# welcomyou/sherpa-vietnamese-asr

Measured on AMD Instinct MI355X. Metric: audio-sec/sec (xRT) Zipformer-68M offline decode, higher is better.
Workload: dtype bf16; 1 GPU; zipformer-68m greedy_search, batched planner chunks, 1 h per GPU; model=zipformer-68m, weights=greedy-calibrated, chunks_per_gpu=121, batch_pipeline=True, encoder_frames_per_gpu=98813

## Files before the change

include/zasr.h:

```cpp
#ifndef ZASR_H_
#define ZASR_H_

#include <stdint.h>

#ifdef __cplusplus
extern "C" {
#endif

typedef struct zasr_recognizer zasr_recognizer;
typedef struct zasr_result zasr_result;

enum {
  ZASR_OK = 0,
  ZASR_ERR_INVALID = 1,
  ZASR_ERR_NOT_FOUND = 2,
  ZASR_ERR_RUNTIME = 3,
};

enum {
  ZASR_PRECISION_FP32 = 0,
  ZASR_PRECISION_BF16 = 1,
  ZASR_PRECISION_BF16_ENC = 2,
  ZASR_PRECISION_BF16X3 = 3,
  ZASR_PRECISION_BF16X6 = 4,
// ... 115 lines not shown

typedef struct zasr_audio zasr_audio;
enum { ZASR_AUDIO_F32 = 0, ZASR_AUDIO_I16 = 1 };
int zasr_audio_create(int32_t device_id, zasr_audio** out);
void zasr_audio_destroy(zasr_audio* h);
int64_t zasr_audio_out_len(int32_t rate, int64_t n_frames);
int zasr_audio_resample_taps(int32_t rate, int32_t* P, int32_t* Q, int32_t* taps,
                             int32_t* out_tile, int32_t* in_tile, int32_t* lo, float* w,
                             int64_t cap);
int zasr_audio_to_16k(zasr_audio* h, const void* src, int32_t format, int32_t channels,
                      int32_t rate, int64_t n_frames, int32_t src_on_device, float* d_out,
                      int64_t cap, int64_t* n_out, void* stream);
int zasr_audio_peak(zasr_audio* h, const float* d_wav, int64_t n, float* peak, void* stream);
int zasr_audio_scale(zasr_audio* h, float* d_wav, int64_t n, float divisor, float multiplier,
                     void* stream);
int zasr_audio_segment_sumsq(zasr_audio* h, const float* d_wav, int64_t n,
                             const int64_t* seg_begin, const int64_t* seg_end, int32_t n_seg,
                             double* out, void* stream);
int zasr_audio_apply_gain(zasr_audio* h, float* d_wav, int64_t n, const int64_t* piece_begin,
                          const int64_t* piece_end, const float* piece_gain,
                          const int64_t* piece_ramp, int32_t n_pieces, const float* ramp_values,
                          int64_t n_ramp_values, float* peak, void* stream);

int32_t zasr_vocab_size(const zasr_recognizer* h);
int32_t zasr_joiner_dim(const zasr_recognizer* h);
int zasr_model_routes(zasr_recognizer* h, char* buf, int64_t cap);
int zasr_fbank_set_mel_banks(zasr_recognizer* h, const float* banks, int32_t n_bins);
int zasr_selftest_launch(int32_t block_threads);
int zasr_selftest_gemm_h3r(int32_t M, int32_t K, int32_t N, int32_t epi, const float* A,
                           const float* W, const float* bias, float* C);
int zasr_selftest_ffn_h3(int32_t R, int32_t D, int32_t F, const float* Y, const float* W1,
                         const float* b1, const float* W2, const float* b2,
                         const float* byp_orig, const float* byp_scale, float* X);
int zasr_selftest_gemm(int32_t mode, int32_t M, int32_t K, int32_t N, int32_t epi, int32_t a_bf16,
                       int32_t c_bf16, const float* A, const float* W, const float* bias,
                       const float* aux, const float* byp_orig, const float* byp_scale, float* C);
int zasr_selftest_ffn_bf16(int32_t R, int32_t D, int32_t F, const float* W1, const float* b1,
                           const float* W2, const float* b2, const float* byp_orig,
                           const float* byp_scale, float* X, int32_t form);
int zasr_selftest_ffn_bf16_oop(int32_t R, int32_t D, int32_t F, const float* W1, const float* b1,
                               const float* W2, const float* b2, const float* byp_orig,
                               const float* byp_scale, float* X, float* Xout, int32_t form);
int zasr_selftest_ffn_h3_oop(int32_t R, int32_t D, int32_t F, const float* W1, const float* b1,
                             const float* W2, const float* b2, const float* byp_orig,
                             const float* byp_scale, float* X, float* Xout);
int zasr_selftest_seam(int32_t nseq, const int32_t* L, int32_t d, int32_t ds, int32_t dn,
                       int32_t ds_next, int32_t c0, int32_t ldo, const float* xd,
                       const float* orig, const float* s, const float* wn8, const float* wo2,
                       float* next, float* xnext, float* out, float* next_ref, float* xnext_ref,
                       float* out_ref);
int zasr_selftest_dwconv1d(int32_t nseq, const int32_t* L, int32_t d, int32_t K, int32_t glu,
                           int32_t bf16, const float* x, const float* w, const float* b,
                           float* out);
int zasr_selftest_conv1(int32_t nseq, const int32_t* T, int32_t form, const float* fb,
                        const float* w, const float* b, float* out);
int zasr_selftest_convnext(int32_t nseq, const int32_t* L, int32_t form, const float* x,
                           const float* dw_w, const float* dw_b, const float* w1, const float* b1,
                           const float* w2, const float* b2, float* y, float* out);
int zasr_selftest_bias_norm(int32_t rows, int32_t d, const float* bias, float log_scale,
                            float* orig, const float* bscale, int32_t copy_mode, float* x,
                            float* copy_out);
int zasr_selftest_attn_block_map(const int32_t* lens, int32_t nseq, int32_t units_per_seq,
                                 int32_t order, uint32_t* out, int64_t cap, int32_t* grid);

typedef struct zasr_diar zasr_diar;
int zasr_diar_create(int32_t device_id, zasr_diar** out);
void zasr_diar_destroy(zasr_diar* h);
int zasr_diar_similarity(zasr_diar* h, const float* d_X, int32_t N, int32_t D, float* d_M,
                         void* stream);
int zasr_diar_prune(zasr_diar* h, float* d_M, int32_t N, double pval, int32_t min_pnum,
                    double* d_deg, void* stream);
int zasr_diar_eigs(zasr_diar* h, const float* d_M, const double* d_deg, int32_t N, int32_t k,
                   double* lambdas, double* vecs, int32_t* passes, void* stream);
int zasr_diar_spectral_embed(zasr_diar* h, const float* X, int32_t x_on_device, int32_t N,
                             int32_t D, double pval, int32_t min_pnum, int32_t k,
                             double* lambdas, double* vecs, void* stream);
int zasr_diar_last_stats(zasr_diar* h, int32_t* passes, int64_t* applications);

int zasr_profile_enable(zasr_recognizer* h, int32_t on);
int zasr_profile_reset(zasr_recognizer* h);
int zasr_profile_report(zasr_recognizer* h, char* buf, int64_t cap);

const char* zasr_last_error(void);
const char* zasr_version(void);

#ifdef __cplusplus
}
#endif
#endif
```

sherpa-vietnamese-asr_amd/csrc/encoder_kernels.hip:

```cpp
#include "common.h"
#include "kernels.h"

namespace zasr {

typedef float f32x16 __attribute__((ext_vector_type(16)));

__device__ __forceinline__ int find_seq(const int* off, int nseq, int r) {
  int lo = 0, hi = nseq - 1;
  while (lo < hi) {
    int mid = (lo + hi + 1) >> 1;
    if (off[mid] <= r) lo = mid;
    else hi = mid - 1;
  }
  return lo;
}

__global__ void row2seq_kernel(const int* __restrict__ off, int nseq, int total,
                               int* __restrict__ map) {
  int r = blockIdx.x * blockDim.x + threadIdx.x;
  if (r < total) map[r] = find_seq(off, nseq, r);
}

void launch_row2seq(const int* off, int nseq, int total, int* map, hipStream_t st) {
  if (total <= 0) return;
// ... 532 lines not shown
    }
  }
  if (tid < kDw1T) {
    const int r = r0 + tid;
    int lo = -half, hi = half;
    if (r < total_rows) {
      lo = max(seq_lo - r, -half);
      hi = min(seq_hi - 1 - r, half);
    }
    sLo[tid] = lo;
    sHi[tid] = hi;
    if (lo != -half || hi != half) atomicOr(&sMasked, 1);
  }
  __syncthreads();
  if (c0 + c >= d) return;
  const int tr0 = (tid >> 6) * 16;
  float acc[16];
#pragma unroll
  for (int i = 0; i < 16; ++i) acc[i] = bc;
  if (!sMasked) {
#pragma unroll
    for (int rr = 0; rr < 16 + K - 1; ++rr) {
      const float v = tile[(tr0 + rr) * 64 + c];
#pragma unroll
      for (int i = 0; i < 16; ++i) {
        const int k = rr - i;
        if (k >= 0 && k < K) acc[i] = fmaf(wr[k], v, acc[i]);
      }
    }
  } else {
    int lo[16], hi[16];
#pragma unroll
    for (int i = 0; i < 16; ++i) {
      lo[i] = sLo[tr0 + i];
      hi[i] = sHi[tr0 + i];
    }
#pragma unroll
    for (int rr = 0; rr < 16 + K - 1; ++rr) {
      const float v = tile[(tr0 + rr) * 64 + c];
#pragma unroll
      for (int i = 0; i < 16; ++i) {
        const int k = rr - i;
        if (k >= 0 && k < K && k - half >= lo[i] && k - half <= hi[i]) acc[i] = fmaf(wr[k], v, acc[i]);
      }
    }
  }
#pragma unroll
  for (int i = 0; i < 16; ++i) {
    const int r = r0 + tr0 + i;
    if (r < total_rows) st1(out + (long)r * d + c0 + c, swooshr_fast(acc[i]));
  }
}

template <typename TI, typename TO, bool GLU = true>
static void launch_glu_dwconv1d_t(const TI* x2, const int* off, const int* map, int total_rows,
                                  int d, int K, const float* w, const float* b, TO* out,
                                  hipStream_t st) {
  if (total_rows <= 0) return;
  ZASR_REQUIRE(d % 4 == 0, "conv module channels must be a multiple of 4");
  dim3 grid(cdiv(total_rows, kDw1T), cdiv(d, 64));
  ZASR_REQUIRE(K >= 1 && K <= 31 && (K & 1), "depthwise kernel size must be odd and <= 31");
  if (K <= 7)
    ZASR_LAUNCH((glu_dwconv1d_kernel<7, TI, TO, GLU>), grid, dim3(256), 0, st, x2, off, map, total_rows, d, K, w, b, out);
  else if (K <= 15)
    ZASR_LAUNCH((glu_dwconv1d_kernel<15, TI, TO, GLU>), grid, dim3(256), 0, st, x2, off, map, total_rows, d, K, w, b, out);
  else
    ZASR_LAUNCH((glu_dwconv1d_kernel<31, TI, TO, GLU>), grid, dim3(256), 0, st, x2, off, map, total_rows, d, K, w, b, out);
}

void launch_dwconv1d_post_glu(const float* g, const int* off, const int* map, int total_rows,
                              int d, int K, const float* w, const float* b, float* out,
                              hipStream_t st) {
  launch_glu_dwconv1d_t<float, float, false>(g, off, map, total_rows, d, K, w, b, out, st);
}

void launch_dwconv1d_post_glu_bf16(const void* g, const int* off, const int* map,
                                   int total_rows, int d, int K, const float* w, const float* b,
                                   void* out, hipStream_t st) {
  launch_glu_dwconv1d_t<__bf16, __bf16, false>(reinterpret_cast<const __bf16*>(g), off, map,
                                               total_rows, d, K, w, b,
                                               reinterpret_cast<__bf16*>(out), st);
}

void launch_glu_dwconv1d(const float* x2, const int* off, const int* map, int total_rows, int d,
                         int K, const float* w, const float* b, float* out, hipStream_t st) {
  launch_glu_dwconv1d_t(x2, off, map, total_rows, d, K, w, b, out, st);
}

struct DsW {
  float w[8];
};

template <int DS>
__global__ void downsample_kernel(const float* __restrict__ x, const int* __restrict__ off_in,
                                  const int* __restrict__ off_out, const int* __restrict__ map_out,
                                  int total_out,
                                  int d4, int ds, DsW wts, float* __restrict__ out) {
  const int e = blockIdx.x * blockDim.x + threadIdx.x;
  if (e >= total_out * d4) return;
  const int r = e / d4, c4 = e - r * d4;
  const int b = map_out[r];
  const int tp = r - off_out[b];
  const int base = off_in[b];
  const int L = off_in[b + 1] - base;
  const float4* x4 = reinterpret_cast<const float4*>(x);
  constexpr int NL = DS > 0 ? DS : 8;
  const int f = DS > 0 ? DS : ds;
  float4 xv[NL];
#pragma unroll
  for (int u = 0; u < NL; ++u) {
    int t = tp * f + (u < f ? u : 0);
    if (t > L - 1) t = L - 1;
    xv[u] = x4[(base + t) * d4 + c4];
  }
  float4 acc = make_float4(0.f, 0.f, 0.f, 0.f);
#pragma unroll
  for (int u = 0; u < NL; ++u)
    if (u < f) {
      acc.x = fmaf(wts.w[u], xv[u].x, acc.x);
      acc.y = fmaf(wts.w[u], xv[u].y, acc.y);
      acc.z = fmaf(wts.w[u], xv[u].z, acc.z);
      acc.w = fmaf(wts.w[u], xv[u].w, acc.w);
    }
  reinterpret_cast<float4*>(out)[e] = acc;
}

void launch_downsample(const float* x, const int* off_in, const int* off_out, const int* map_out,
                       int total_out, int d, int ds, const float* w_host8, float* out,
                       hipStream_t st) {
  const long n = (long)total_out * (d / 4);
  if (n <= 0) return;
  ZASR_REQUIRE(d % 4 == 0 && n < (1L << 31), "downsample: width must be a multiple of 4");
  DsW w{};
  for (int i = 0; i < ds && i < 8; ++i) w.w[i] = w_host8[i];
// ... 619 lines not shown
```

sherpa-vietnamese-asr_amd/csrc/kernels.h:

```cpp
#pragma once
#include <cstdint>
#include <vector>

#include <hip/hip_runtime.h>

namespace zasr {

struct FbankTables {
  const double* twiddle;
  const float* window;
  const int* mel_start;
  const int* mel_len;
  const int* mel_woff;
  const float* mel_w;
};
void launch_fbank(const float* wav, const long* wav_off, const int* nsamp, const int* fr_off,
                  int nseq, int total_frames, const FbankTables& tabs, float* out,
                  hipStream_t st, bool campp = false);

void launch_silence_flags(const float* wav, long n, int frame_len, float threshold,
                          unsigned char* flags, hipStream_t st);

void launch_selftest_noop(int block_threads);
void selftest_gemm_h3r(int M, int K, int N, int epi, const float* A, const float* W,
// ... 77 lines not shown
  float* frames;
  int n_files;
};
void launch_vad_maxabs(const float* audio, const long* off, const long* len, int n_files,
                       unsigned* mx, hipStream_t st);
void launch_vad_frames(const VadFramesArgs& a, long n_windows, hipStream_t st);
void launch_vad_mag_im2col(const float* S, int ldS, int bins, int Kp, long n_windows, float* A,
                           hipStream_t st);
void launch_vad_im2col(const float* Y, long N, int T, int C, int stride, int Tout, float* A,
                       hipStream_t st);
struct VadLstmArgs {
  const float* gx;
  const float* whh;
  const float* bhh;
  const float* wd;
  float bd;
  const long* seg_start;
  const int* seg_count;
  const int* seg_warm;
  const float* init;
  float* s_out;
  float* e_out;
  float* probs;
};
void launch_vad_lstm(const VadLstmArgs& a, int n_segments, hipStream_t st);

void launch_conv1(const float* fb, const int* fb_off, const int* c1_off, const int* c1_map,
                  int total_rows, const float* w , const float* b, void* out,
                  bool out_bf16, hipStream_t st, bool fast = false);
void pack_frag32_host(const __bf16* w, int rows, int cols, __bf16* out);
void launch_convnext_bf16(const void* x, const int* L_off, const int* L_map, int total_rows,
                          const float* dw_w, const float* dw_b, const void* w1, const float* b1,
                          const void* w2, const float* b2, void* ytmp, void* out,
                          hipStream_t st);
void launch_convnext_mlp_h3(const float* y, const float* x, long npos, const void* w1p,
                            const float* b1, const void* w2p, const float* b2, float* out,
                            hipStream_t st);
void launch_dwconv2d_tiled(const float* x, const int* L_off, const int* L_map, int total_rows,
                           const float* w, const float* b, float* out, hipStream_t st);

void selftest_seam(int nseq, const int* L, int d, int ds, int dn, int ds_next, int c0, int ldo,
                   const float* xd, const float* orig, const float* s, const float* wn8,
                   const float* wo2, float* next, float* xnext, float* out, float* next_ref,
                   float* xnext_ref, float* out_ref);
void launch_bias_norm(float* x, int rows, int d, const float* bias, float log_scale,
                      const float* orig, const float* bypass_scale, hipStream_t st,
                      float* copy_out = nullptr);
void launch_bypass(float* x, const float* orig, const float* s, long rows, int d, hipStream_t st);
void launch_glu(const float* x2, float* g, long rows, int d, hipStream_t st);
void launch_glu_dwconv1d(const float* x2, const int* off, const int* map, int total_rows, int d,
                         int K, const float* w, const float* b, float* out, hipStream_t st);
void launch_dwconv1d_post_glu(const float* g, const int* off, const int* map, int total_rows,
                              int d, int K, const float* w, const float* b, float* out,
                              hipStream_t st);
void launch_dwconv1d_post_glu_bf16(const void* g, const int* off, const int* map,
                                   int total_rows, int d, int K, const float* w, const float* b,
                                   void* out, hipStream_t st);
void launch_nonlin_prep(const float* h3, float* t1, long rows, int hid, hipStream_t st);
void launch_downsample(const float* x, const int* off_in, const int* off_out, const int* map_out,
                       int total_out, int d, int ds, const float* w_host8, float* out,
                       hipStream_t st);
void launch_upsample_combine(const float* xd, const float* orig, const int* off_in,
                             const int* off_ds, const int* map_in, int total_rows, int d, int ds,
                             const float* s, float* y, hipStream_t st);
void launch_stack_glue(const float* xd, const float* orig, const int* off_in, const int* off_ds,
                       const int* map_in, int rows, int d, int ds, const float* s, float* next,
                       int dn, float* full, int ldf, int c0, hipStream_t st);
struct SeamDesc {
  const float* xd = nullptr;
  const float* orig = nullptr;
  const float* s = nullptr;
  const int* off_in = nullptr;
  const int* off_ds = nullptr;
  const int* off_run = nullptr;
  const int* map_run = nullptr;
  int runs = 0;
  int rows = 0;
  int d = 0, ds = 1;
  float* next = nullptr;
  int dn = 0;
  int ds_next = 1;
  float* xnext = nullptr;
  const float* wn_host8 = nullptr;
  float* out = nullptr;
  const int* off_out = nullptr;
  const float* wo_host2 = nullptr;
  int ldo = 0, c0 = 0;
};
void launch_seam(const SeamDesc& s, hipStream_t st);
void selftest_dwconv1d(int nseq, const int* L, int d, int K, bool glu, bool bf16, const float* x,
                       const float* w, const float* b, float* out);
void selftest_conv1(int nseq, const int* T, int form, const float* fb, const float* w,
                    const float* b, float* out);
void selftest_convnext(int nseq, const int* L, int form, const float* x, const float* dw_w,
                       const float* dw_b, const float* w1, const float* b1, const float* w2,
                       const float* b2, float* y, float* out);
void selftest_bias_norm(int rows, int d, const float* bias, float log_scale, float* orig,
                        const float* bscale, int copy_mode, float* x, float* copy_out);
void launch_row2seq(const int* off, int nseq, int total, int* map, hipStream_t st);
void launch_copy_cols(const float* src, int lds, int c0, float* dst, int ldd, int d0, int ncols,
                      long rows, bool zero_rest, int dst_width, hipStream_t st);

struct AttnArgs {
  const float* qkp;
  int H;
  const float* pos_tab;
  int pmax;
  const int* row_off;
  const long* a_off;
  int nseq;
  int max_len;
  float* attn;
  float* stats;
  int write_heads;
};
void launch_attn_softmax(const AttnArgs& a, hipStream_t st);
struct AttnFlashArgs {
  const void* qkp;
  int H;
  const float* pos_tab;
  int pmax;
  const int* row_off;
  const long* a_off;
  int nseq;
  int max_len;
  void* attn;
  const void* v;
  void* out;
  const float* stats_in;
  float* stats_out;
  int pieces = 1;
  const void* t1t = nullptr;
  const int* o8 = nullptr;
  int ldt = 0;
  int hid = 0;
  const void* y = nullptr;
  int ldy = 0;
  void* z = nullptr;
  const unsigned* map = nullptr;
  int map_len = 0;
};
void launch_attn_flash(const AttnFlashArgs& a, int mode, hipStream_t st);
inline int attn_nonlin_frags(int hid, int pieces) {
  const int nft = (hid + 31) / 32;
// ... 185 lines not shown
```

sherpa-vietnamese-asr_amd/csrc/selftest.cpp:

```cpp
#include <cstring>
#include <memory>
#include <vector>

#include "../../include/zasr.h"
#include "common.h"
#include "dense_gemm.h"
#include "gemm.h"
#include "kernels.h"

namespace zasr {
namespace {
struct DevBuf {
  void* p = nullptr;
  explicit DevBuf(size_t bytes) { ZASR_HIP_CHECK(hipMalloc(&p, bytes > 0 ? bytes : 4)); }
  ~DevBuf() { (void)hipFree(p); }
  template <class T>
  T* as() const { return reinterpret_cast<T*>(p); }
};
void up(DevBuf& d, const void* h, size_t bytes) {
  if (bytes) ZASR_HIP_CHECK(hipMemcpy(d.p, h, bytes, hipMemcpyHostToDevice));
}
}

void selftest_gemm_h3r(int M, int K, int N, int epi, const float* A, const float* W,
// ... 275 lines not shown
  DevBuf d_off, d_map;
  Level(int nseq, const int* len, int cut)
      : off(offsets(nseq, len, cut)), rows(off.back()), d_off(off.size() * 4),
        d_map((size_t)rows * 4) {
    up(d_off, off.data(), off.size() * 4);
    launch_row2seq(d_off.as<int>(), nseq, rows, d_map.as<int>(), nullptr);
  }
  static std::vector<int> offsets(int nseq, const int* len, int cut) {
    ZASR_REQUIRE(nseq >= 1 && len != nullptr, "selftest: at least one sequence");
    std::vector<int> o(nseq + 1, 0);
    for (int b = 0; b < nseq; ++b) {
      ZASR_REQUIRE(len[b] - cut >= 1, "selftest: every sequence needs a frame at every level");
      o[b + 1] = o[b] + len[b] - cut;
    }
    return o;
  }
};

struct OutBuf {
  size_t n, row, eb;
  DevBuf d;
  OutBuf(const float* init, size_t n_, size_t row_, bool h16)
      : n(n_), row(row_), eb(h16 ? 2 : 4), d((n_ + row_) * (h16 ? 2 : 4)) {
    if (h16) up(d, round16(init, n).data(), n * 2);
    else up(d, init, n * 4);
    ZASR_HIP_CHECK(hipMemset(d.as<unsigned char>() + n * eb, 0x5a, row * eb));
  }
  template <class T>
  T* as() const { return d.as<T>(); }
  void down(float* out, const char* what) const {
    std::vector<unsigned char> guard(row * eb);
    ZASR_HIP_CHECK(hipMemcpy(guard.data(), d.as<unsigned char>() + n * eb, guard.size(),
                             hipMemcpyDeviceToHost));
    for (unsigned char g : guard)
      ZASR_REQUIRE(g == 0x5a, std::string("selftest ") + what + ": the kernel wrote past the last row");
    if (n == 0) return;
    if (eb == 2) {
      std::vector<__bf16> h(n);
      ZASR_HIP_CHECK(hipMemcpy(h.data(), d.p, n * 2, hipMemcpyDeviceToHost));
      for (size_t i = 0; i < n; ++i) out[i] = (float)h[i];
    } else {
      ZASR_HIP_CHECK(hipMemcpy(out, d.p, n * 4, hipMemcpyDeviceToHost));
    }
  }
};

void up16(DevBuf& d, const float* h, size_t n, bool h16) {
  if (h16) up(d, round16(h, n).data(), n * 2);
  else up(d, h, n * 4);
}
}

void selftest_dwconv1d(int nseq, const int* L, int d, int K, bool glu, bool bf16, const float* x,
                       const float* w, const float* b, float* out) {
  ZASR_REQUIRE(!(glu && bf16), "selftest dwconv1d: the GLU form is f32 only");
  ZASR_REQUIRE(d >= 4 && d % 4 == 0, "selftest dwconv1d: d a positive multiple of 4");
  ZASR_REQUIRE(K >= 1 && K <= 31 && (K & 1), "selftest dwconv1d: K odd, at most 31");
  Level lv(nseq, L, 0);
  const size_t nx = (size_t)lv.rows * (glu ? 2 * d : d), no = (size_t)lv.rows * d;
  DevBuf dX(nx * (bf16 ? 2 : 4)), dW((size_t)d * K * 4), dB((size_t)d * 4);
  up16(dX, x, nx, bf16);
  up(dW, w, (size_t)d * K * 4);
  up(dB, b, (size_t)d * 4);
  OutBuf o(out, no, d, bf16);
  if (glu)
    launch_glu_dwconv1d(dX.as<float>(), lv.d_off.as<int>(), lv.d_map.as<int>(), lv.rows, d, K,
                        dW.as<float>(), dB.as<float>(), o.as<float>(), nullptr);
  else if (bf16)
    launch_dwconv1d_post_glu_bf16(dX.p, lv.d_off.as<int>(), lv.d_map.as<int>(), lv.rows, d, K,
                                  dW.as<float>(), dB.as<float>(), o.d.p, nullptr);
  else
    launch_dwconv1d_post_glu(dX.as<float>(), lv.d_off.as<int>(), lv.d_map.as<int>(), lv.rows, d, K,
                             dW.as<float>(), dB.as<float>(), o.as<float>(), nullptr);
  ZASR_HIP_CHECK(hipDeviceSynchronize());
  o.down(out, "dwconv1d");
}

void selftest_conv1(int nseq, const int* T, int form, const float* fb, const float* w,
                    const float* b, float* out) {
  ZASR_REQUIRE(form >= 0 && form <= 2, "selftest conv1: form 0 (libm), 1 (fast) or 2 (bf16 out)");
  Level lf(nseq, T, 0), lc(nseq, T, 2);
  DevBuf dF((size_t)lf.rows * 80 * 4), dW(8 * 9 * 4), dB(8 * 4);
  up(dF, fb, (size_t)lf.rows * 80 * 4);
  up(dW, w, 8 * 9 * 4);
  up(dB, b, 8 * 4);
  OutBuf o(out, (size_t)lc.rows * 640, 640, form == 2);
  launch_conv1(dF.as<float>(), lf.d_off.as<int>(), lc.d_off.as<int>(), lc.d_map.as<int>(), lc.rows,
               dW.as<float>(), dB.as<float>(), o.d.p, form == 2, nullptr, form == 1);
  ZASR_HIP_CHECK(hipDeviceSynchronize());
  o.down(out, "conv1");
}

void selftest_convnext(int nseq, const int* L, int form, const float* x, const float* dw_w,
                       const float* dw_b, const float* w1, const float* b1, const float* w2,
                       const float* b2, float* y, float* out) {
  ZASR_REQUIRE(form >= 0 && form <= 2,
               "selftest convnext: form 0 (depthwise f32), 1 (bf16 block) or 2 (f16x3 block)");
  ZASR_REQUIRE(form == 0 || (w1 && b1 && w2 && b2 && out), "selftest convnext: the MLP's operands");
  Level lv(nseq, L, 0);
  constexpr size_t kRow = 19 * 128, kW = 384 * 128;
  const size_t n = (size_t)lv.rows * kRow;
  const bool h16 = form == 1;
  DevBuf dWd(128 * 49 * 4), dBd(128 * 4), d1(2 * kW * 2), d2(2 * kW * 2), db1(384 * 4), db2(128 * 4);
  up(dWd, dw_w, 128 * 49 * 4);
  up(dBd, dw_b, 128 * 4);
  OutBuf oy(y, n, kRow, h16);
  const int *off = lv.d_off.as<int>(), *map = lv.d_map.as<int>();
  if (form == 0) {
    DevBuf dX(n * 4);
    up(dX, x, n * 4);
    launch_dwconv2d_tiled(dX.as<float>(), off, map, lv.rows, dWd.as<float>(), dBd.as<float>(),
                          oy.as<float>(), nullptr);
    ZASR_HIP_CHECK(hipDeviceSynchronize());
    oy.down(y, "convnext");
    return;
  }
  up(db1, b1, 384 * 4);
  up(db2, b2, 128 * 4);
  auto pack = [&](const float* wsrc, int rows, int cols, DevBuf& dst) {
    std::vector<__bf16> img(2 * kW), piece(kW);
    if (h16) {
      pack_frag32_host(round16(wsrc, kW).data(), rows, cols, img.data());
    } else {
      for (int t = 0; t < 2; ++t) {
        for (size_t i = 0; i < kW; ++i) {
          const _Float16 hi = (_Float16)wsrc[i];
// ... 57 lines not shown
```

sherpa-vietnamese-asr_amd/csrc/zasr_api.cpp:

```cpp
#include <cstdio>
#include <cstring>
#include <fstream>
#include <memory>
#include <mutex>
#include <sstream>
#include <string>
#include <vector>

#include "../../include/zasr.h"
#include "audio.h"
#include "campp.h"
#include "common.h"
#include "diar.h"
#include "vad.h"
#include "vibert.h"
#include "engine.h"
#include "host_io.h"
#include "onnx_io.h"

using zasr::Engine;
using zasr::TokenResult;

struct zasr_recognizer {
  std::unique_ptr<Engine> eng;
// ... 672 lines not shown
                           const float* byp_scale, float* X, int32_t form) {
  if (!W1 || !b1 || !W2 || !b2 || !X) return fail(ZASR_ERR_INVALID, "null argument");
  return guarded([&]() {
    zasr::selftest_ffn_bf16(R, D, F, W1, b1, W2, b2, byp_orig, byp_scale, X, form);
    return (int)ZASR_OK;
  });
}

int zasr_selftest_ffn_bf16_oop(int32_t R, int32_t D, int32_t F, const float* W1, const float* b1,
                               const float* W2, const float* b2, const float* byp_orig,
                               const float* byp_scale, float* X, float* Xout, int32_t form) {
  if (!W1 || !b1 || !W2 || !b2 || !X || !Xout) return fail(ZASR_ERR_INVALID, "null argument");
  return guarded([&]() {
    zasr::selftest_ffn_bf16(R, D, F, W1, b1, W2, b2, byp_orig, byp_scale, X, form, Xout);
    return (int)ZASR_OK;
  });
}

int zasr_selftest_ffn_h3_oop(int32_t R, int32_t D, int32_t F, const float* W1, const float* b1,
                             const float* W2, const float* b2, const float* byp_orig,
                             const float* byp_scale, float* X, float* Xout) {
  if (!W1 || !b1 || !W2 || !b2 || !X || !Xout) return fail(ZASR_ERR_INVALID, "null argument");
  return guarded([&]() {
    zasr::selftest_ffn_h3(R, D, F, nullptr, W1, b1, W2, b2, byp_orig, byp_scale, X, Xout);
    return (int)ZASR_OK;
  });
}

int zasr_selftest_seam(int32_t nseq, const int32_t* L, int32_t d, int32_t ds, int32_t dn,
                       int32_t ds_next, int32_t c0, int32_t ldo, const float* xd,
                       const float* orig, const float* s, const float* wn8, const float* wo2,
                       float* next, float* xnext, float* out, float* next_ref, float* xnext_ref,
                       float* out_ref) {
  if (!L || !orig || !wn8 || !wo2 || !next || !xnext || !out || !next_ref || !xnext_ref ||
      !out_ref || (ds > 1 && (!xd || !s)))
    return fail(ZASR_ERR_INVALID, "null argument");
  return guarded([&]() {
    zasr::selftest_seam(nseq, L, d, ds, dn, ds_next, c0, ldo, xd, orig, s, wn8, wo2, next, xnext,
                        out, next_ref, xnext_ref, out_ref);
    return (int)ZASR_OK;
  });
}

int zasr_selftest_dwconv1d(int32_t nseq, const int32_t* L, int32_t d, int32_t K, int32_t glu,
                           int32_t bf16, const float* x, const float* w, const float* b,
                           float* out) {
  if (!L || !x || !w || !b || !out) return fail(ZASR_ERR_INVALID, "null argument");
  return guarded([&]() {
    zasr::selftest_dwconv1d(nseq, L, d, K, glu != 0, bf16 != 0, x, w, b, out);
    return (int)ZASR_OK;
  });
}

int zasr_selftest_conv1(int32_t nseq, const int32_t* T, int32_t form, const float* fb,
                        const float* w, const float* b, float* out) {
  if (!T || !fb || !w || !b || !out) return fail(ZASR_ERR_INVALID, "null argument");
  return guarded([&]() {
    zasr::selftest_conv1(nseq, T, form, fb, w, b, out);
    return (int)ZASR_OK;
  });
}

int zasr_selftest_convnext(int32_t nseq, const int32_t* L, int32_t form, const float* x,
                           const float* dw_w, const float* dw_b, const float* w1, const float* b1,
                           const float* w2, const float* b2, float* y, float* out) {
  if (!L || !x || !dw_w || !dw_b || !y) return fail(ZASR_ERR_INVALID, "null argument");
  return guarded([&]() {
    zasr::selftest_convnext(nseq, L, form, x, dw_w, dw_b, w1, b1, w2, b2, y, out);
    return (int)ZASR_OK;
  });
}

int zasr_selftest_bias_norm(int32_t rows, int32_t d, const float* bias, float log_scale,
                            float* orig, const float* bscale, int32_t copy_mode, float* x,
                            float* copy_out) {
  if (!bias || !x) return fail(ZASR_ERR_INVALID, "null argument");
  return guarded([&]() {
    zasr::selftest_bias_norm(rows, d, bias, log_scale, orig, bscale, copy_mode, x, copy_out);
    return (int)ZASR_OK;
  });
}

int zasr_selftest_attn_block_map(const int32_t* lens, int32_t nseq, int32_t units_per_seq,
                                 int32_t order, uint32_t* out, int64_t cap, int32_t* grid) {
  if (!lens || !grid || (cap > 0 && !out) || cap < 0) return fail(ZASR_ERR_INVALID, "null argument");
  return guarded([&]() {
    std::vector<unsigned> map;
    *grid = zasr::build_attn_block_map(lens, nseq, units_per_seq, order, map);
    if ((int64_t)map.size() > cap) return fail(ZASR_ERR_INVALID, "block map buffer too small");
    std::copy(map.begin(), map.end(), out);
    return (int)ZASR_OK;
  });
}

int zasr_silence_flags(const float* d_wav, int64_t n, int32_t frame_len, float threshold,
                       uint8_t* d_flags, void* stream) {
  if (n < 0 || (n > 0 && (!d_wav || !d_flags))) return fail(ZASR_ERR_INVALID, "null argument");
  return guarded([&]() {
    zasr::launch_silence_flags(d_wav, (long)n, (int)frame_len, threshold, d_flags,
                               reinterpret_cast<hipStream_t>(stream));
    return (int)ZASR_OK;
  });
}

namespace {
int audio_source_error(int32_t format, int32_t channels, int32_t rate) {
// ... 349 lines not shown
```

sherpa-vietnamese-asr_amd/zasr/binding.py:

```python
from __future__ import annotations

import ctypes as C
import dataclasses
import os
from typing import List, Optional, Sequence

import numpy as np

_PKG = os.path.dirname(os.path.dirname(os.path.abspath(__file__)))
DEFAULT_LIB = os.path.join(_PKG, "lib", "libzasr.so")

EXPORTS = (
    "zasr_create", "zasr_destroy", "zasr_convert_model", "zasr_convert_stage_model", "zasr_fbank", "zasr_decode_batch", "zasr_decode_features",
    "zasr_decode_device", "zasr_decode_device_batches", "zasr_encode_features", "zasr_search_encoder_out",
    "zasr_result_count", "zasr_result_num_tokens", "zasr_result_num_frames",
    "zasr_result_tokens", "zasr_result_frames", "zasr_result_log_probs",
    "zasr_result_token_stats", "zasr_result_free", "zasr_vocab_size", "zasr_joiner_dim",
    "zasr_profile_enable", "zasr_profile_reset", "zasr_profile_report", "zasr_last_error",
    "zasr_version", "zasr_campp_create", "zasr_campp_destroy", "zasr_campp_embedding_dim",
    "zasr_campp_fbank", "zasr_campp_embed", "zasr_campp_embed_device", "zasr_campp_windows_device",
    "zasr_vibert_create", "zasr_vibert_destroy", "zasr_vibert_num_labels",
    "zasr_vibert_num_detect", "zasr_vibert_run",
    "zasr_vad_create", "zasr_vad_destroy", "zasr_vad_probs", "zasr_vad_probs_device",
    "zasr_vad_window", "zasr_vad_last_passes", "zasr_silence_flags",
    "zasr_create_stream", "zasr_destroy_stream", "zasr_stream_accept_waveform",
    "zasr_decode_stream", "zasr_decode_streams", "zasr_stream_is_decoded",
    "zasr_stream_num_tokens", "zasr_stream_num_frames", "zasr_stream_tokens",
    "zasr_stream_frames", "zasr_stream_log_probs", "zasr_stream_token_stats",
    "zasr_stream_result_json", "zasr_set_tokens", "zasr_model_routes",
    "zasr_fbank_set_mel_banks", "zasr_selftest_launch", "zasr_decode_host_batches",
    "zasr_selftest_gemm_h3r", "zasr_selftest_ffn_h3", "zasr_selftest_ffn_bf16",
    "zasr_selftest_attn_block_map", "zasr_selftest_seam", "zasr_selftest_ffn_bf16_oop",
    "zasr_selftest_ffn_h3_oop", "zasr_selftest_gemm",
    "zasr_selftest_dwconv1d", "zasr_selftest_conv1", "zasr_selftest_convnext",
    "zasr_selftest_bias_norm",
    "zasr_audio_create", "zasr_audio_destroy", "zasr_audio_out_len", "zasr_audio_resample_taps",
    "zasr_audio_to_16k", "zasr_audio_peak", "zasr_audio_scale", "zasr_audio_segment_sumsq",
    "zasr_audio_apply_gain",
    "zasr_diar_create", "zasr_diar_destroy", "zasr_diar_similarity", "zasr_diar_prune",
    "zasr_diar_eigs", "zasr_diar_spectral_embed", "zasr_diar_last_stats",
)


PRECISIONS = {"fp32": 0, "bf16": 1, "bf16_enc": 2, "bf16x3": 3, "bf16x6": 4, "f16x3": 5}


C_FP = C.POINTER(C.c_float)


class ZasrError(RuntimeError):
    pass


class _Config(C.Structure):
    _fields_ = [
        ("model_dir", C.c_char_p),
        ("decoding_method", C.c_char_p),
        ("max_active_paths", C.c_int32),
        ("blank_penalty", C.c_float),
        ("hotword_tokens", C.POINTER(C.c_int32)),
        ("hotword_lens", C.POINTER(C.c_int32)),
        ("hotword_scores", C.POINTER(C.c_float)),
        ("num_hotwords", C.c_int32),
        ("device_id", C.c_int32),
        ("precision", C.c_int32),
    ]


_lib = None


def load_library(path: Optional[str] = None) -> C.CDLL:
    global _lib
    if _lib is not None and path is None:
        return _lib
    p = path or os.environ.get("ZASR_LIB", DEFAULT_LIB)
    if not os.path.exists(p):
        raise ZasrError(f"libzasr.so not found at {p}; build it with "
                        f"`make -C sherpa-vietnamese-asr_amd/csrc` (or __graft_entry__.build())")
    lib = C.CDLL(p)
    P, I32, I64 = C.c_void_p, C.c_int32, C.c_int64
    fp = C.POINTER(C.c_float)
    lib.zasr_create.argtypes = [C.POINTER(_Config), C.POINTER(P)]
    lib.zasr_create.restype = C.c_int
    lib.zasr_destroy.argtypes = [P]
    lib.zasr_destroy.restype = None
    lib.zasr_convert_model.argtypes = [C.c_char_p, C.c_char_p]
    lib.zasr_convert_model.restype = C.c_int
# ... 90 lines not shown
    lib.zasr_vad_last_passes.restype = I32
    lib.zasr_silence_flags.argtypes = [P, I64, I32, C.c_float, P, P]
    lib.zasr_silence_flags.restype = C.c_int
    lib.zasr_create_stream.argtypes = [P, C.POINTER(P)]
    lib.zasr_create_stream.restype = C.c_int
    lib.zasr_destroy_stream.argtypes = [P]
    lib.zasr_destroy_stream.restype = None
    lib.zasr_stream_accept_waveform.argtypes = [P, I32, fp, I64]
    lib.zasr_stream_accept_waveform.restype = C.c_int
    lib.zasr_decode_stream.argtypes = [P, P]
    lib.zasr_decode_stream.restype = C.c_int
    lib.zasr_decode_streams.argtypes = [P, C.POINTER(P), I32]
    lib.zasr_decode_streams.restype = C.c_int
    for n in ("zasr_stream_is_decoded", "zasr_stream_num_tokens", "zasr_stream_num_frames"):
        getattr(lib, n).argtypes = [P]
        getattr(lib, n).restype = I32
    lib.zasr_stream_tokens.argtypes = [P]
    lib.zasr_stream_tokens.restype = C.POINTER(I32)
    lib.zasr_stream_frames.argtypes = [P]
    lib.zasr_stream_frames.restype = C.POINTER(I32)
    lib.zasr_stream_log_probs.argtypes = [P]
    lib.zasr_stream_log_probs.restype = C.POINTER(C.c_double)
    lib.zasr_stream_token_stats.argtypes = [P]
    lib.zasr_stream_token_stats.restype = fp
    lib.zasr_stream_result_json.argtypes = [P, C.c_char_p, I64, C.POINTER(I64)]
    lib.zasr_stream_result_json.restype = C.c_int
    lib.zasr_set_tokens.argtypes = [P, C.c_char_p]
    lib.zasr_set_tokens.restype = C.c_int
    lib.zasr_model_routes.argtypes = [P, C.c_char_p, I64]
    lib.zasr_model_routes.restype = C.c_int
    lib.zasr_fbank_set_mel_banks.argtypes = [P, fp, I32]
    lib.zasr_fbank_set_mel_banks.restype = C.c_int
    lib.zasr_selftest_launch.argtypes = [I32]
    lib.zasr_selftest_launch.restype = C.c_int
    lib.zasr_selftest_gemm_h3r.argtypes = [I32, I32, I32, I32, fp, fp, fp, fp]
    lib.zasr_selftest_gemm_h3r.restype = C.c_int
    lib.zasr_selftest_gemm.argtypes = [I32] * 7 + [fp] * 7
    lib.zasr_selftest_gemm.restype = C.c_int
    lib.zasr_selftest_ffn_h3.argtypes = [I32, I32, I32, fp, fp, fp, fp, fp, fp, fp, fp]
    lib.zasr_selftest_ffn_h3.restype = C.c_int
    lib.zasr_selftest_ffn_bf16.argtypes = [I32, I32, I32, fp, fp, fp, fp, fp, fp, fp, I32]
    lib.zasr_selftest_ffn_bf16.restype = C.c_int
    lib.zasr_selftest_attn_block_map.argtypes = [C.POINTER(I32), I32, I32, I32,
                                                 C.POINTER(C.c_uint32), I64, C.POINTER(I32)]
    lib.zasr_selftest_attn_block_map.restype = C.c_int
    lib.zasr_selftest_seam.argtypes = [I32, C.POINTER(I32)] + [I32] * 6 + [fp] * 11
    lib.zasr_selftest_seam.restype = C.c_int
    lib.zasr_selftest_ffn_bf16_oop.argtypes = [I32, I32, I32] + [fp] * 8 + [I32]
    lib.zasr_selftest_ffn_bf16_oop.restype = C.c_int
    lib.zasr_selftest_ffn_h3_oop.argtypes = [I32, I32, I32] + [fp] * 8
    lib.zasr_selftest_ffn_h3_oop.restype = C.c_int
    lib.zasr_selftest_dwconv1d.argtypes = [I32, C.POINTER(I32)] + [I32] * 4 + [fp] * 4
    lib.zasr_selftest_dwconv1d.restype = C.c_int
    lib.zasr_selftest_conv1.argtypes = [I32, C.POINTER(I32), I32] + [fp] * 4
    lib.zasr_selftest_conv1.restype = C.c_int
    lib.zasr_selftest_convnext.argtypes = [I32, C.POINTER(I32), I32] + [fp] * 9
    lib.zasr_selftest_convnext.restype = C.c_int
    lib.zasr_selftest_bias_norm.argtypes = [I32, I32, fp, C.c_float, fp, fp, I32, fp, fp]
    lib.zasr_selftest_bias_norm.restype = C.c_int
    lib.zasr_audio_create.argtypes = [I32, C.POINTER(P)]
    lib.zasr_audio_create.restype = C.c_int
    lib.zasr_audio_destroy.argtypes = [P]
    lib.zasr_audio_destroy.restype = None
    lib.zasr_audio_out_len.argtypes = [I32, I64]
    lib.zasr_audio_out_len.restype = I64
    lib.zasr_audio_resample_taps.argtypes = [I32, i32p, i32p, i32p, i32p, i32p, i32p, fp, I64]
    lib.zasr_audio_resample_taps.restype = C.c_int
    lib.zasr_audio_to_16k.argtypes = [P, P, I32, I32, I32, I64, I32, P, I64, i64p, P]
    lib.zasr_audio_to_16k.restype = C.c_int
    lib.zasr_audio_peak.argtypes = [P, P, I64, fp, P]
    lib.zasr_audio_peak.restype = C.c_int
    lib.zasr_audio_scale.argtypes = [P, P, I64, C.c_float, C.c_float, P]
    lib.zasr_audio_scale.restype = C.c_int
    lib.zasr_audio_segment_sumsq.argtypes = [P, P, I64, i64p, i64p, I32, C.POINTER(C.c_double), P]
    lib.zasr_audio_segment_sumsq.restype = C.c_int
    lib.zasr_audio_apply_gain.argtypes = [P, P, I64, i64p, i64p, fp, i64p, I32, fp, I64, fp, P]
    lib.zasr_audio_apply_gain.restype = C.c_int
    dp, DBL = C.POINTER(C.c_double), C.c_double
    lib.zasr_diar_create.argtypes = [I32, C.POINTER(P)]
    lib.zasr_diar_create.restype = C.c_int
    lib.zasr_diar_destroy.argtypes = [P]
    lib.zasr_diar_destroy.restype = None
    lib.zasr_diar_similarity.argtypes = [P, P, I32, I32, P, P]
    lib.zasr_diar_similarity.restype = C.c_int
    lib.zasr_diar_prune.argtypes = [P, P, I32, DBL, I32, P, P]
    lib.zasr_diar_prune.restype = C.c_int
    lib.zasr_diar_eigs.argtypes = [P, P, P, I32, I32, dp, dp, i32p, P]
    lib.zasr_diar_eigs.restype = C.c_int
    lib.zasr_diar_spectral_embed.argtypes = [P, P, I32, I32, I32, DBL, I32, I32, dp, dp, P]
    lib.zasr_diar_spectral_embed.restype = C.c_int
    lib.zasr_diar_last_stats.argtypes = [P, i32p, i64p]
    lib.zasr_diar_last_stats.restype = C.c_int
    if path is None:
        _lib = lib
    return lib


def convert_model(model_dir: str, out_dir: str, lib_path: Optional[str] = None) -> None:
    lib = load_library(lib_path)
    os.makedirs(out_dir, exist_ok=True)
    rc = lib.zasr_convert_model(model_dir.encode(), out_dir.encode())
    if rc != 0:
        msg = lib.zasr_last_error().decode()
        if rc == 2:
            raise FileNotFoundError(msg)
        raise ZasrError(msg)
# ... 93 lines not shown
def selftest_ffn_oop(kind: str, W1, b1, W2, b2, X, byp_orig=None, byp_scale=None, form: int = 0,
                     fill: float = -777.25, lib_path: Optional[str] = None):
    lib = load_library(lib_path)
    W1, b1, W2, b2, X = (_f32(v) for v in (W1, b1, W2, b2, X))
    X = X.copy()
    out = np.full(X.shape, fill, dtype=np.float32)
    bo = None if byp_orig is None else _f32(byp_orig)
    bs = None if byp_scale is None else _f32(byp_scale)
    p = lambda x: None if x is None else x.ctypes.data_as(C_FP)
    args = (X.shape[0], X.shape[1], W1.shape[0], p(W1), p(b1), p(W2), p(b2), p(bo), p(bs), p(X),
            p(out))
    if kind == "bf16":
        rc = lib.zasr_selftest_ffn_bf16_oop(*args, int(form))
    elif kind == "h3":
        rc = lib.zasr_selftest_ffn_h3_oop(*args)
    else:
        raise ValueError(kind)
    if rc != 0:
        raise ZasrError(lib.zasr_last_error().decode())
    return out, X


def selftest_seam(L, d: int, ds: int, dn: int, ds_next: int, c0: int, ldo: int, xd, orig, s,
                  wn8, wo2, fill: float = -777.25, lib_path: Optional[str] = None) -> dict:
    lib = load_library(lib_path)
    L = np.ascontiguousarray(L, dtype=np.int32)
    orig, wn8, wo2 = _f32(orig), _f32(wn8), _f32(wo2)
    xd = None if xd is None else _f32(xd)
    s = None if s is None else _f32(s)
    rows = int(L.sum())
    rn = int(((L + ds_next - 1) // ds_next).sum())
    ro = int(((L + 1) // 2).sum())
    assert orig.shape == (rows, d) and wn8.shape == (8,) and wo2.shape == (2,)
    assert ds == 1 or (xd.shape == (int(((L + ds - 1) // ds).sum()), d) and s.shape == (d,))
    res = {}
    for name, shape in (("next", (rows, dn)), ("xnext", (rn, dn)), ("out", (ro, ldo))):
        for k in (name, name + "_ref"):
            res[k] = np.full(shape, fill, dtype=np.float32)
    p = lambda x: None if x is None else x.ctypes.data_as(C_FP)
    rc = lib.zasr_selftest_seam(len(L), L.ctypes.data_as(C.POINTER(C.c_int32)), int(d), int(ds),
                                int(dn), int(ds_next), int(c0), int(ldo), p(xd), p(orig), p(s),
                                p(wn8), p(wo2), p(res["next"]), p(res["xnext"]), p(res["out"]),
                                p(res["next_ref"]), p(res["xnext_ref"]), p(res["out_ref"]))
    if rc != 0:
        raise ZasrError(lib.zasr_last_error().decode())
    return res


def _lens(L) -> np.ndarray:
    return np.ascontiguousarray(L, dtype=np.int32)


def selftest_dwconv1d(L, x, w, b, glu: bool, bf16: bool = False, fill: float = -777.25,
                      lib_path: Optional[str] = None) -> np.ndarray:
    lib = load_library(lib_path)
    L, x, w, b = _lens(L), _f32(x), _f32(w), _f32(b)
    rows, (d, K) = int(L.sum()), w.shape
    assert x.shape == (rows, 2 * d if glu else d) and b.shape == (d,)
    out = np.full((rows, d), fill, dtype=np.float32)
    p = lambda a: a.ctypes.data_as(C_FP)
    rc = lib.zasr_selftest_dwconv1d(len(L), L.ctypes.data_as(C.POINTER(C.c_int32)), d, K,
                                    int(glu), int(bf16), p(x), p(w), p(b), p(out))
    if rc != 0:
        raise ZasrError(lib.zasr_last_error().decode())
    return out


def selftest_conv1(T, fb, w, b, form: int, fill: float = -777.25,
                   lib_path: Optional[str] = None) -> np.ndarray:
    lib = load_library(lib_path)
    T, fb, w, b = _lens(T), _f32(fb), _f32(w), _f32(b)
    assert fb.shape == (int(T.sum()), 80) and w.shape == (8, 9) and b.shape == (8,)
    out = np.full((int((T - 2).sum()), 80, 8), fill, dtype=np.float32)
    p = lambda a: a.ctypes.data_as(C_FP)
    rc = lib.zasr_selftest_conv1(len(T), T.ctypes.data_as(C.POINTER(C.c_int32)), int(form), p(fb),
                                 p(w), p(b), p(out))
    if rc != 0:
        raise ZasrError(lib.zasr_last_error().decode())
    return out


def selftest_convnext(L, x, dw_w, dw_b, w1=None, b1=None, w2=None, b2=None, form: int = 0,
                      fill: float = -777.25, lib_path: Optional[str] = None):
    lib = load_library(lib_path)
    L, x, dw_w, dw_b = _lens(L), _f32(x), _f32(dw_w), _f32(dw_b)
    rows = int(L.sum())
    assert x.shape == (rows, 19, 128) and dw_w.shape == (128, 7, 7) and dw_b.shape == (128,)
    mlp = [None if v is None else _f32(v) for v in (w1, b1, w2, b2)]
    if form != 0:
        assert [v.shape for v in mlp] == [(384, 128), (384,), (128, 384), (128,)]
    y = np.full(x.shape, fill, dtype=np.float32)
    out = None if form == 0 else np.full(x.shape, fill, dtype=np.float32)
    p = lambda a: None if a is None else a.ctypes.data_as(C_FP)
    rc = lib.zasr_selftest_convnext(len(L), L.ctypes.data_as(C.POINTER(C.c_int32)), int(form),
                                    p(x), p(dw_w), p(dw_b), *(p(v) for v in mlp), p(y), p(out))
    if rc != 0:
        raise ZasrError(lib.zasr_last_error().decode())
    return y, out


def selftest_bias_norm(x, bias, log_scale: float, orig=None, bscale=None, copy_mode: int = 0,
                       fill: float = -777.25, lib_path: Optional[str] = None) -> dict:
    lib = load_library(lib_path)
    x, bias = _f32(x).copy(), _f32(bias)
    rows, d = x.shape
    o = None if orig is None else _f32(orig).copy()
    s = None if bscale is None else _f32(bscale)
    cp = np.full(x.shape, fill, dtype=np.float32) if copy_mode == 1 else None
    p = lambda a: None if a is None else a.ctypes.data_as(C_FP)
    rc = lib.zasr_selftest_bias_norm(rows, d, p(bias), float(log_scale), p(o), p(s),
                                     int(copy_mode), p(x), p(cp))
    if rc != 0:
        raise ZasrError(lib.zasr_last_error().decode())
    return {"x": x, "orig": o, "copy": cp}

# ... 646 lines not shown
```

Before: 134,800 audio-sec/sec.

## Add DMA-staged depthwise conv1d kernel for post-GLU path

Adds a new depthwise conv1d kernel for the post-GLU, same-type case that stages the input tile into LDS with global_load_lds (direct global-to-LDS DMA) instead of going through registers. Each wave computes 16 rows and takes a fast unmasked path when the whole window lies inside one sequence, falling back to zero-fill or per-row bounds only near sequence edges. It becomes the default whenever d is a multiple of 64, and the old kernel stays reachable through a form selector exposed in the selftest API. The aim is to cut load latency and per-tap boundary checks in the conv module, at the cost of more code paths and reliance on a low-level builtin plus manual vmcnt waits.

```diff
diff --git a/include/zasr.h b/include/zasr.h
--- a/include/zasr.h
+++ b/include/zasr.h
@@ -191,6 +191,9 @@
 int zasr_selftest_dwconv1d(int32_t nseq, const int32_t* L, int32_t d, int32_t K, int32_t glu,
                            int32_t bf16, const float* x, const float* w, const float* b,
                            float* out);
+int zasr_selftest_dwconv1d_form(int32_t nseq, const int32_t* L, int32_t d, int32_t K, int32_t glu,
+                                int32_t bf16, const float* x, const float* w, const float* b,
+                                float* out, int32_t form);
 int zasr_selftest_conv1(int32_t nseq, const int32_t* T, int32_t form, const float* fb,
                         const float* w, const float* b, float* out);
 int zasr_selftest_convnext(int32_t nseq, const int32_t* L, int32_t form, const float* x,
diff --git a/sherpa-vietnamese-asr_amd/csrc/encoder_kernels.hip b/sherpa-vietnamese-asr_amd/csrc/encoder_kernels.hip
--- a/sherpa-vietnamese-asr_amd/csrc/encoder_kernels.hip
+++ b/sherpa-vietnamese-asr_amd/csrc/encoder_kernels.hip
@@ -608,14 +608,165 @@
   }
 }
 
+typedef __attribute__((address_space(3))) void* dw1_lds_t;
+
+__device__ __forceinline__ float dw1_widen(float v) { return v; }
+__device__ __forceinline__ float dw1_widen(__bf16 v) {
+  return __builtin_bit_cast(float, (unsigned)__builtin_bit_cast(unsigned short, v) << 16);
+}
+
+__device__ __forceinline__ void dw1_glds16(const void* g, unsigned char* lds_base) {
+  __builtin_amdgcn_global_load_lds(const_cast<void*>(g), (dw1_lds_t)(lds_base), 16, 0, 0);
+}
+__device__ __forceinline__ void dw1_wait_vm0() { asm volatile("s_waitcnt vmcnt(0)" ::: "memory"); }
+__device__ __forceinline__ int dw1_wave(int tid) { return __builtin_amdgcn_readfirstlane(tid >> 6) & 3; }
+
+template <int K, bool ZF, typename T>
+__device__ __forceinline__ void dw1_chain(const T* col, const float (&wr)[K], float (&acc)[16],
+                                          int rfirst, int lo, int hi) {
+#pragma unroll
+  for (int rr = 0; rr < 16 + K - 1; ++rr) {
+    float v = dw1_widen(col[rr * 64]);
+    if constexpr (ZF) {
+      const int r = rfirst + rr;
+      v = (r >= lo && r < hi) ? v : 0.f;
+    }
+#pragma unroll
+    for (int i = 0; i < 16; ++i) {
+      const int k = rr - i;
+      if (k >= 0 && k < K) acc[i] = fmaf(wr[k], v, acc[i]);
+    }
+  }
+}
+
+template <int K, typename T>
+__global__ __launch_bounds__(256) void dwconv1d_dma_kernel(
+    const T* __restrict__ x, const int* __restrict__ off, const int* __restrict__ map,
+    int total_rows, int d, int Kr, const float* __restrict__ w, const float* __restrict__ bias,
+    T* __restrict__ out) {
+  constexpr int half = K / 2;
+  constexpr int nrows = kDw1T + K - 1;
+  constexpr int kPR = 1024 / (64 * (int)sizeof(T));
+  constexpr int kLPR = 64 / kPR;
+  constexpr int kEPL = 16 / (int)sizeof(T);
+  constexpr int nP = (nrows + kPR - 1) / kPR;
+  constexpr int kPIt = (nP + 3) / 4;
+  constexpr int kTileB = nP * 1024;
+  __shared__ __attribute__((aligned(16))) unsigned char smem[kTileB + 64 * K * 4];
+  const T* tile = reinterpret_cast<const T*>(smem);
+  float* sW = reinterpret_cast<float*>(smem + kTileB);
+  const int r0 = blockIdx.x * kDw1T;
+  const int c0 = blockIdx.y * 64;
+  const int tid = threadIdx.x;
+  const int c = tid & 63;
+  const int wid = dw1_wave(tid);
+  const int nw = 64 * Kr;
+  constexpr int kWIt = (64 * K + 255) / 256;
+  float wl[kWIt];
+#pragma unroll
+  for (int q = 0; q < kWIt; ++q) {
+    const int i = tid + 256 * q;
+    wl[q] = w[(long)c0 * Kr + (i < nw ? i : nw - 1)];
+  }
+  const float bc = bias[c0 + c];
+#pragma unroll
+  for (int q = 0; q < kPIt; ++q) {
+    const int p = wid + 4 * q;
+    if (p < nP) {
+      int r = r0 - half + p * kPR + c / kLPR;
+      r = r < 0 ? 0 : (r >= total_rows ? total_rows - 1 : r);
+      dw1_glds16(x + (long)r * d + c0 + (c % kLPR) * kEPL, smem + p * 1024);
+    }
+  }
+  const int g0 = r0 + wid * 16;
+  const int gl = min(g0 + 15, total_rows - 1);
+  const int b0 = map[min(g0, total_rows - 1)], b1 = map[gl];
+  const int lo = off[b0], hi = off[b0 + 1];
+  dw1_wait_vm0();
+#pragma unroll
+  for (int q = 0; q < kWIt; ++q) {
+    const int i = tid + 256 * q;
+    if (i < nw) sW[i] = wl[q];
+  }
+  __syncthreads();
+  if (g0 >= total_rows) return;
+  float wr[K];
+  if (Kr == K) {
+#pragma unroll
+    for (int k = 0; k < K; ++k) wr[k] = sW[c * K + k];
+  } else {
+    const int pad = (K - Kr) / 2;
+#pragma unroll
+    for (int k = 0; k < K; ++k) {
+      const int kk = k - pad;
+      const bool ok = kk >= 0 && kk < Kr;
+      const float wv = sW[c * Kr + (ok ? kk : 0)];
+      wr[k] = ok ? wv : 0.f;
+    }
+  }
+  float acc[16];
+#pragma unroll
+  for (int i = 0; i < 16; ++i) acc[i] = bc;
+  const T* col = tile + wid * 16 * 64 + c;
+  if (b0 == b1) {
+    if (g0 - half >= lo && gl + half < hi)
+      dw1_chain<K, false>(col, wr, acc, g0 - half, lo, hi);
+    else
+      dw1_chain<K, true>(col, wr, acc, g0 - half, lo, hi);
+  } else {
+    int tlo[16], thi[16];
+#pragma unroll
+    for (int i = 0; i < 16; ++i) {
+      const int r = g0 + i;
+      const int b = map[min(r, total_rows - 1)];
+      tlo[i] = max(off[b] - r, -half);
+      thi[i] = min(off[b + 1] - 1 - r, half);
+    }
+#pragma unroll
+    for (int rr = 0; rr < 16 + K - 1; ++rr) {
+      const float v = dw1_widen(col[rr * 64]);
+#pragma unroll
+      for (int i = 0; i < 16; ++i) {
+        const int k = rr - i;
+        if (k >= 0 && k < K && k - half >= tlo[i] && k - half <= thi[i]) acc[i] = fmaf(wr[k], v, acc[i]);
+      }
+    }
+  }
+#pragma unroll
+  for (int i = 0; i < 16; ++i) acc[i] = swooshr_fast(acc[i]);
+  T* o = out + (long)g0 * d + c0 + c;
+  if (g0 + 15 < total_rows) {
+#pragma unroll
+    for (int i = 0; i < 16; ++i) st1(o + (long)i * d, acc[i]);
+  } else {
+#pragma unroll
+    for (int i = 0; i < 16; ++i)
+      if (g0 + i < total_rows) st1(o + (long)i * d, acc[i]);
+  }
+}
+
 template <typename TI, typename TO, bool GLU = true>
 static void launch_glu_dwconv1d_t(const TI* x2, const int* off, const int* map, int total_rows,
                                   int d, int K, const float* w, const float* b, TO* out,
-                                  hipStream_t st) {
+                                  hipStream_t st, int form = -1) {
   if (total_rows <= 0) return;
   ZASR_REQUIRE(d % 4 == 0, "conv module channels must be a multiple of 4");
   dim3 grid(cdiv(total_rows, kDw1T), cdiv(d, 64));
   ZASR_REQUIRE(K >= 1 && K <= 31 && (K & 1), "depthwise kernel size must be odd and <= 31");
+  constexpr bool can_dma = !GLU && std::is_same<TI, TO>::value;
+  ZASR_REQUIRE(form != 1 || (can_dma && d % 64 == 0),
+               "dwconv1d: the DMA form needs a post-GLU input and d a multiple of 64");
+  if constexpr (can_dma) {
+    if (form != 0 && d % 64 == 0) {
+      if (K <= 7)
+        ZASR_LAUNCH((dwconv1d_dma_kernel<7, TI>), grid, dim3(256), 0, st, x2, off, map, total_rows, d, K, w, b, out);
+      else if (K <= 15)
+        ZASR_LAUNCH((dwconv1d_dma_kernel<15, TI>), grid, dim3(256), 0, st, x2, off, map, total_rows, d, K, w, b, out);
+      else
+        ZASR_LAUNCH((dwconv1d_dma_kernel<31, TI>), grid, dim3(256), 0, st, x2, off, map, total_rows, d, K, w, b, out);
+      return;
+    }
+  }
   if (K <= 7)
     ZASR_LAUNCH((glu_dwconv1d_kernel<7, TI, TO, GLU>), grid, dim3(256), 0, st, x2, off, map, total_rows, d, K, w, b, out);
   else if (K <= 15)
@@ -626,16 +777,16 @@
 
 void launch_dwconv1d_post_glu(const float* g, const int* off, const int* map, int total_rows,
                               int d, int K, const float* w, const float* b, float* out,
-                              hipStream_t st) {
-  launch_glu_dwconv1d_t<float, float, false>(g, off, map, total_rows, d, K, w, b, out, st);
+                              hipStream_t st, int form) {
+  launch_glu_dwconv1d_t<float, float, false>(g, off, map, total_rows, d, K, w, b, out, st, form);
 }
 
 void launch_dwconv1d_post_glu_bf16(const void* g, const int* off, const int* map,
                                    int total_rows, int d, int K, const float* w, const float* b,
-                                   void* out, hipStream_t st) {
+                                   void* out, hipStream_t st, int form) {
   launch_glu_dwconv1d_t<__bf16, __bf16, false>(reinterpret_cast<const __bf16*>(g), off, map,
                                                total_rows, d, K, w, b,
-                                               reinterpret_cast<__bf16*>(out), st);
+                                               reinterpret_cast<__bf16*>(out), st, form);
 }
 
 void launch_glu_dwconv1d(const float* x2, const int* off, const int* map, int total_rows, int d,
diff --git a/sherpa-vietnamese-asr_amd/csrc/kernels.h b/sherpa-vietnamese-asr_amd/csrc/kernels.h
--- a/sherpa-vietnamese-asr_amd/csrc/kernels.h
+++ b/sherpa-vietnamese-asr_amd/csrc/kernels.h
@@ -153,10 +153,10 @@
                          int K, const float* w, const float* b, float* out, hipStream_t st);
 void launch_dwconv1d_post_glu(const float* g, const int* off, const int* map, int total_rows,
                               int d, int K, const float* w, const float* b, float* out,
-                              hipStream_t st);
+                              hipStream_t st, int form = -1);
 void launch_dwconv1d_post_glu_bf16(const void* g, const int* off, const int* map,
                                    int total_rows, int d, int K, const float* w, const float* b,
-                                   void* out, hipStream_t st);
+                                   void* out, hipStream_t st, int form = -1);
 void launch_nonlin_prep(const float* h3, float* t1, long rows, int hid, hipStream_t st);
 void launch_downsample(const float* x, const int* off_in, const int* off_out, const int* map_out,
                        int total_out, int d, int ds, const float* w_host8, float* out,
@@ -190,7 +190,7 @@
 };
 void launch_seam(const SeamDesc& s, hipStream_t st);
 void selftest_dwconv1d(int nseq, const int* L, int d, int K, bool glu, bool bf16, const float* x,
-                       const float* w, const float* b, float* out);
+                       const float* w, const float* b, float* out, int form = -1);
 void selftest_conv1(int nseq, const int* T, int form, const float* fb, const float* w,
                     const float* b, float* out);
 void selftest_convnext(int nseq, const int* L, int form, const float* x, const float* dw_w,
diff --git a/sherpa-vietnamese-asr_amd/csrc/selftest.cpp b/sherpa-vietnamese-asr_amd/csrc/selftest.cpp
--- a/sherpa-vietnamese-asr_amd/csrc/selftest.cpp
+++ b/sherpa-vietnamese-asr_amd/csrc/selftest.cpp
@@ -351,8 +351,10 @@
 }
 
 void selftest_dwconv1d(int nseq, const int* L, int d, int K, bool glu, bool bf16, const float* x,
-                       const float* w, const float* b, float* out) {
+                       const float* w, const float* b, float* out, int form) {
   ZASR_REQUIRE(!(glu && bf16), "selftest dwconv1d: the GLU form is f32 only");
+  ZASR_REQUIRE(form >= -1 && form <= 1, "selftest dwconv1d: form 0 or 1");
+  ZASR_REQUIRE(!(glu && form == 1), "selftest dwconv1d: the DMA form takes a post-GLU input");
   ZASR_REQUIRE(d >= 4 && d % 4 == 0, "selftest dwconv1d: d a positive multiple of 4");
   ZASR_REQUIRE(K >= 1 && K <= 31 && (K & 1), "selftest dwconv1d: K odd, at most 31");
   Level lv(nseq, L, 0);
@@ -367,10 +369,10 @@
                         dW.as<float>(), dB.as<float>(), o.as<float>(), nullptr);
   else if (bf16)
     launch_dwconv1d_post_glu_bf16(dX.p, lv.d_off.as<int>(), lv.d_map.as<int>(), lv.rows, d, K,
-                                  dW.as<float>(), dB.as<float>(), o.d.p, nullptr);
+                                  dW.as<float>(), dB.as<float>(), o.d.p, nullptr, form);
   else
     launch_dwconv1d_post_glu(dX.as<float>(), lv.d_off.as<int>(), lv.d_map.as<int>(), lv.rows, d, K,
-                             dW.as<float>(), dB.as<float>(), o.as<float>(), nullptr);
+                             dW.as<float>(), dB.as<float>(), o.as<float>(), nullptr, form);
   ZASR_HIP_CHECK(hipDeviceSynchronize());
   o.down(out, "dwconv1d");
 }
diff --git a/sherpa-vietnamese-asr_amd/csrc/zasr_api.cpp b/sherpa-vietnamese-asr_amd/csrc/zasr_api.cpp
--- a/sherpa-vietnamese-asr_amd/csrc/zasr_api.cpp
+++ b/sherpa-vietnamese-asr_amd/csrc/zasr_api.cpp
@@ -748,6 +748,17 @@
   });
 }
 
+int zasr_selftest_dwconv1d_form(int32_t nseq, const int32_t* L, int32_t d, int32_t K, int32_t glu,
+                                int32_t bf16, const float* x, const float* w, const float* b,
+                                float* out, int32_t form) {
+  if (!L || !x || !w || !b || !out) return fail(ZASR_ERR_INVALID, "null argument");
+  if (form != 0 && form != 1) return fail(ZASR_ERR_INVALID, "form is 0 or 1");
+  return guarded([&]() {
+    zasr::selftest_dwconv1d(nseq, L, d, K, glu != 0, bf16 != 0, x, w, b, out, form);
+    return (int)ZASR_OK;
+  });
+}
+
 int zasr_selftest_conv1(int32_t nseq, const int32_t* T, int32_t form, const float* fb,
                         const float* w, const float* b, float* out) {
   if (!T || !fb || !w || !b || !out) return fail(ZASR_ERR_INVALID, "null argument");
diff --git a/sherpa-vietnamese-asr_amd/zasr/binding.py b/sherpa-vietnamese-asr_amd/zasr/binding.py
--- a/sherpa-vietnamese-asr_amd/zasr/binding.py
+++ b/sherpa-vietnamese-asr_amd/zasr/binding.py
@@ -33,7 +33,7 @@
     "zasr_selftest_attn_block_map", "zasr_selftest_seam", "zasr_selftest_ffn_bf16_oop",
     "zasr_selftest_ffn_h3_oop", "zasr_selftest_gemm",
     "zasr_selftest_dwconv1d", "zasr_selftest_conv1", "zasr_selftest_convnext",
-    "zasr_selftest_bias_norm",
+    "zasr_selftest_bias_norm", "zasr_selftest_dwconv1d_form",
     "zasr_audio_create", "zasr_audio_destroy", "zasr_audio_out_len", "zasr_audio_resample_taps",
     "zasr_audio_to_16k", "zasr_audio_peak", "zasr_audio_scale", "zasr_audio_segment_sumsq",
     "zasr_audio_apply_gain",
@@ -230,6 +230,8 @@
     lib.zasr_selftest_ffn_h3_oop.restype = C.c_int
     lib.zasr_selftest_dwconv1d.argtypes = [I32, C.POINTER(I32)] + [I32] * 4 + [fp] * 4
     lib.zasr_selftest_dwconv1d.restype = C.c_int
+    lib.zasr_selftest_dwconv1d_form.argtypes = [I32, C.POINTER(I32)] + [I32] * 4 + [fp] * 4 + [I32]
+    lib.zasr_selftest_dwconv1d_form.restype = C.c_int
     lib.zasr_selftest_conv1.argtypes = [I32, C.POINTER(I32), I32] + [fp] * 4
     lib.zasr_selftest_conv1.restype = C.c_int
     lib.zasr_selftest_convnext.argtypes = [I32, C.POINTER(I32), I32] + [fp] * 9
@@ -429,15 +431,19 @@
 
 
 def selftest_dwconv1d(L, x, w, b, glu: bool, bf16: bool = False, fill: float = -777.25,
-                      lib_path: Optional[str] = None) -> np.ndarray:
+                      lib_path: Optional[str] = None, form: Optional[int] = None) -> np.ndarray:
     lib = load_library(lib_path)
     L, x, w, b = _lens(L), _f32(x), _f32(w), _f32(b)
     rows, (d, K) = int(L.sum()), w.shape
     assert x.shape == (rows, 2 * d if glu else d) and b.shape == (d,)
     out = np.full((rows, d), fill, dtype=np.float32)
     p = lambda a: a.ctypes.data_as(C_FP)
-    rc = lib.zasr_selftest_dwconv1d(len(L), L.ctypes.data_as(C.POINTER(C.c_int32)), d, K,
-                                    int(glu), int(bf16), p(x), p(w), p(b), p(out))
+    args = (len(L), L.ctypes.data_as(C.POINTER(C.c_int32)), d, K, int(glu), int(bf16), p(x), p(w),
+            p(b), p(out))
+    if form is None:
+        rc = lib.zasr_selftest_dwconv1d(*args)
+    else:
+        rc = lib.zasr_selftest_dwconv1d_form(*args, int(form))
     if rc != 0:
         raise ZasrError(lib.zasr_last_error().decode())
     return out
```

Result: slower. 132,200 audio-sec/sec (-1.9%).
